# CMU-SAFARI/Genome-on-Diet

Measured on AMD Instinct MI355X. Metric: mapped bases/sec (whole node), HiFi map-hifi k19w19, higher is better.
Workload: dtype int16

## Files before the change

### genome-on-diet_amd/build.py

```python
import os
import re
import subprocess

HERE = os.path.dirname(os.path.abspath(__file__))
LIB = os.path.join(HERE, "libgdiet_hip.so")
SRC = os.path.join(HERE, "csrc", "gdiet_hip.hip")
RES = os.path.join(HERE, "build_resources.txt")

BUDGET = {"_Z21ksw_extd2_wave_kernelILi64ELi0ELb1E": dict(vgprs=96, scratch=0),
          "_Z21ksw_extd2_pipe_kernelILb1E": dict(vgprs=128, scratch=320),
          "_Z20map_post_wave_kernel": dict(vgprs=32, scratch=0),
          "_Z21map_pack_cigar_kernel": dict(vgprs=32, scratch=0),
          "_Z25ksw_backtrack_wave_kernel": dict(vgprs=32, scratch=0),
          "_Z22ksw_exact_match_kernel": dict(vgprs=32, scratch=0),
          "_Z18map_diffstr_kernel": dict(vgprs=32, scratch=0),
          "_Z18fastx_count_kernel": dict(vgprs=32, scratch=0),
          "_Z18fastx_write_kernel": dict(vgprs=32, scratch=0),
          "_Z19fastx_record_kernel": dict(vgprs=32, scratch=0),
          "_Z19fastx_encode_kernel": dict(vgprs=32, scratch=0),
          "_Z19bgzf_inflate_kernel": dict(vgprs=64, scratch=0),
          "_Z19bgzf_deflate_kernel": dict(vgprs=128, scratch=0),
          "_Z17bam_encode_kernel": dict(vgprs=32, scratch=0),
          "_Z17sam_encode_kernel": dict(vgprs=32, scratch=0),
          "_Z17bam_unpack_kernel": dict(vgprs=32, scratch=0),
          "_Z14bam_key_kernel": dict(vgprs=32, scratch=0),
          "_Z17bam_gather_kernel": dict(vgprs=32, scratch=0),
          "_Z14dup_key_kernel": dict(vgprs=32, scratch=0),
          "_Z17dup_decide_kernel": dict(vgprs=32, scratch=0),
          "_Z16dup_apply_kernel": dict(vgprs=32, scratch=0),
          "_Z18cov_scatter_kernel": dict(vgprs=32, scratch=0),
          "_Z17cov_window_kernel": dict(vgprs=32, scratch=0),
          "_Z19pile_scatter_kernel": dict(vgprs=32, scratch=0),
          "_Z16pile_call_kernel": dict(vgprs=32, scratch=0),
          "_Z16pile_site_kernel": dict(vgprs=32, scratch=0)}


def _newest_source():
    m = 0.0
    for root in (os.path.join(HERE, "csrc"), os.path.join(os.path.dirname(HERE), "include")):
        for f in os.listdir(root):
            m = max(m, os.path.getmtime(os.path.join(root, f)))
    return m


def check_resources(text):
    found = {}
    blocks = re.split(r"remark: Function Name: ", text)
    for b in blocks[1:]:
        name = b.split()[0]
        for prefix, lim in BUDGET.items():
            if name.startswith(prefix):
                v = re.search(r"remark:\s+VGPRs: (\d+)", b)
                sc = re.search(r"ScratchSize \[bytes/lane\]: (\d+)", b)
                if v and sc:
                    found[prefix] = (int(v.group(1)), int(sc.group(1)))
                    if int(v.group(1)) > lim["vgprs"] or int(sc.group(1)) > lim["scratch"]:
                        raise RuntimeError("%s: %d VGPRs / %d B scratch per lane, budget %d / %d (genome-on-diet_amd/build.py)"
                                           % (name, int(v.group(1)), int(sc.group(1)), lim["vgprs"], lim["scratch"]))
    missing = [p for p in BUDGET if p not in found]
    if missing:
        raise RuntimeError("no resource report for %s" % missing)
    return found


def build_hip(force=False, verbose=False):
    if not force and os.path.exists(LIB) and os.path.getmtime(LIB) >= _newest_source():
        return LIB
    hipcc = os.environ.get("HIPCC", "/opt/rocm/bin/hipcc")
    cmd = [hipcc, "--offload-arch=gfx950", "-O3", "-std=c++17", "-fPIC", "-shared", "-pthread", "-mllvm", "-amdgpu-sched-strategy=max-ilp",
           "-Rpass-analysis=kernel-resource-usage", "-o", LIB, SRC, "-lz"]
    if verbose:
        print(" ".join(cmd))
    r = subprocess.run(cmd, stderr=subprocess.PIPE, text=True)
    remarks = "\n".join(l for l in r.stderr.split("\n") if "-Rpass-analysis=kernel-resource-usage" in l)
    other = "\n".join(l for l in r.stderr.split("\n") if "-Rpass-analysis=kernel-resource-usage" not in l)
    if r.returncode:
        raise RuntimeError("hipcc failed:\n" + other[-4000:])
    open(RES, "w").write(remarks)
    found = check_resources(remarks)
    if verbose:
        print("register budgets:", found)
    return LIB


if __name__ == "__main__":
    print(build_hip(force=True, verbose=True))
```

### genome-on-diet_amd/csrc/map_kernels.hip.h

```cpp
#pragma once
#include <hip/hip_runtime.h>
#include "map_stages.h"
#include "map_post.h"

struct MapDevOpt {
	int32_t k, w;
	float max_seeds, q_occ_frac;
	int32_t mid_occ, max_max_occ, occ_dist;
	uint32_t max_nb_seeds;
	int64_t flag;
	GdLrVoteOpt vote;
	GdSrVoteOpt sr;
	int32_t is_sr;
	int32_t sort_cap;
	uint32_t seed_lds;
	int32_t prio;
	GdPattern pat;
};
__device__ __forceinline__ void map_set_prio(int p)
{
	if (p == 1) __builtin_amdgcn_s_setprio(1);
	else if (p == 2) __builtin_amdgcn_s_setprio(2);
	else if (p >= 3) __builtin_amdgcn_s_setprio(3);
}


struct MapSeedOut {
	int32_t n_seeds;
	int32_t shift;
	uint32_t tel;
	uint32_t n_mv;
	int64_t n_a;
};

__device__ __forceinline__ unsigned map_sketch2_lds(const uint8_t *str, int len, int w, int k, const GdPattern &P, float max_seeds, GdMini *out, unsigned max_out,
                                                    uint32_t *shift_n, GdMini *win)
{
	unsigned len_crop, total = 0;
	uint32_t cap;
	if (max_seeds < 1) len_crop = (unsigned)((float)max_seeds * len), cap = UINT32_MAX;
	else len_crop = len, cap = (uint32_t)max_seeds;
	for (int shift = 0; shift < P.W; ++shift) {
		const unsigned dl = gd_diet_len(P, len_crop, shift);
		GdEmitCount e = {out + total, 0, cap, max_out - total, false};
		gd_sketch_range<GdEmitCount, true>(str, 0, 0, dl, 0, true, w, k, 0, (unsigned)shift, P, true, e, win, 64);
		if (e.overflow) return ~0u;
		shift_n[shift] = e.n;
		total += e.n;
		if (cap == UINT32_MAX) len_crop = len, cap = e.n;
	}
	return total;
}
__device__ __forceinline__ unsigned map_sketch3_lds(const uint8_t *str, unsigned len, int w, int k, const GdPattern &P, int shift, uint32_t max_nb_seeds, GdMini *out,
                                                    unsigned max_out, unsigned *n_out, GdMini *win)
{
	if (shift < 0) shift = 0;
	const unsigned dl = gd_diet_len(P, len, (unsigned)shift);
	GdEmitCap e = {out, 0, max_nb_seeds, max_out, len, false};
	gd_sketch_range<GdEmitCap, true>(str, 0, 0, dl, 0, true, w, k, 0, (unsigned)shift, P, true, e, win, 64);
	*n_out = e.overflow ? ~0u : e.n;
	return e.ret;
}

__global__ __launch_bounds__(64) void map_seed_kernel(int n_reads, const uint8_t *__restrict__ reads, const int64_t *__restrict__ roff,
                                                      GdIdxView I, MapDevOpt O, const MapReadScratch *__restrict__ sc, GdMini *__restrict__ mv_arena,
                                                      uint64_t *__restrict__ u64_arena, GdSeed *__restrict__ seed_arena, MapSeedOut *__restrict__ out)
{
	extern __shared__ __attribute__((aligned(16))) uint8_t seed_thread_lds[];
	GdMini *win = reinterpret_cast<GdMini *>(seed_thread_lds) + threadIdx.x;
	const int rid = blockIdx.x * blockDim.x + threadIdx.x;
	if (rid >= n_reads) return;
	const uint8_t *str = reads + roff[rid];
	const int len = (int)(roff[rid + 1] - roff[rid]);
	MapSeedOut o;
	o.n_seeds = 0, o.shift = 0, o.tel = (uint32_t)len, o.n_mv = 0, o.n_a = 0;
	if (len <= 0) { out[rid] = o; return; }
	const MapReadScratch S = sc[rid];
	GdMini *mv = mv_arena + S.mv_off;
	uint32_t shift_n[64];
	const unsigned tot = map_sketch2_lds(str, len, O.w, O.k, O.pat, O.max_seeds, mv, S.mv_cap, shift_n, win);
	if (tot == ~0u) { o.n_seeds = -1; out[rid] = o; return; }
	o.shift = (int32_t)gd_get_shift(I, mv, shift_n, O.pat.W);
	unsigned n_mv = 0;
	o.tel = map_sketch3_lds(str, (unsigned)len, O.w, O.k, O.pat, o.shift, O.max_nb_seeds, mv, S.mv_cap, &n_mv, win);
	if (n_mv == ~0u) { o.n_seeds = -1; out[rid] = o; return; }
// ... 313 lines not shown
	GdPostOut P;
	P.qshift = P.tshift = P.mlen = P.blen = P.dp_max = 0, P.n_ambi = 0;
	const int32_t n0 = __builtin_amdgcn_readfirstlane(n_cigar[b]);
	const int32_t sc_b = __builtin_amdgcn_readfirstlane(score[b]);
	const int64_t c0 = coff[b], c1 = coff[b + 1];
	const bool live = sc_b != GD_NEG_INF_SCORE_DEV && n0 > 0 && (int64_t)n0 <= c1 - c0;
	int32_t n_out = n0;
	if (live) {
		uint32_t *cg = (uint32_t *)gdw_uniform_ptr((const uint8_t *)(cig + c0), 0);
		const uint8_t *qseq = gdw_uniform_ptr(qbuf + boxes[b].q_dst, 0), *tseq = gdw_uniform_ptr(tbuf + boxes[b].t_dst, 0);
		uint32_t n_fix = (uint32_t)n0;
		int32_t qshift = 0, tshift = 0;
		if (lane == 0) {
			gdp_fix_cigar(cg, &n_fix, qseq, tseq, &qshift, &tshift);
			n_cigar[b] = (int32_t)n_fix;
		}
		__builtin_amdgcn_fence(__ATOMIC_SEQ_CST, "workgroup");
		const uint32_t n = (uint32_t)__builtin_amdgcn_readfirstlane((int)n_fix);
		n_out = (int32_t)n;
		P.qshift = __builtin_amdgcn_readfirstlane(qshift), P.tshift = __builtin_amdgcn_readfirstlane(tshift);
		__syncthreads();
		qseq += P.qshift, tseq += P.tshift;
		int32_t Si = 0, Sf = 0, MXi = 0, MXf = 0;
		int32_t qoff = 0, toff = 0, blen = 0, mlen = 0;
		uint32_t n_ambi_tot = 0;
		for (uint32_t k = 0; k < n; ++k) {
			const uint32_t c = (uint32_t)__builtin_amdgcn_readfirstlane((int)cg[k]), op = c & 0xf, len = c >> 4;
			if (op == 0) {
				for (uint32_t base = 0; base < len; base += 64) {
					GdpSeg g = {0, GDP_NONE, GDP_NONE, GDP_NONE};
					int cnt2 = 0;
					const uint32_t l = base + lane;
					if (l < len) {
						const int cq = qseq[qoff + l], ct = tseq[toff + l];
						if (ct > 3 || cq > 3) cnt2 = 1;
						else if (ct != cq) cnt2 = 1 << 16;
						const int idx = ct * 5 + cq;
						const int32_t a = idx < 25 ? (int32_t)s_mat[idx] : 0;
						g = gdp_seg_base(a);
					}
#pragma unroll 1
					for (int d = 1; d < 64; d <<= 1) {
						GdpSeg o;
						o.A = __shfl_down(g.A, d), o.B = __shfl_down(g.B, d), o.P = __shfl_down(g.P, d), o.Q = __shfl_down(g.Q, d);
						const int oc = __shfl_down(cnt2, d);
						if (lane + d < 64) g = gdp_seg_join(g, o), cnt2 += oc;
					}
					const int32_t A = __builtin_amdgcn_readfirstlane(g.A), Bc = __builtin_amdgcn_readfirstlane(g.B), Pm = __builtin_amdgcn_readfirstlane(g.P),
					              Qm = __builtin_amdgcn_readfirstlane(g.Q);
					const int c2 = __builtin_amdgcn_readfirstlane(cnt2), na = c2 & 0xffff, nd = c2 >> 16;
					gdp_run_fold(A, Bc, Pm, Qm, Si, Sf, MXi, MXf);
					const uint32_t cnt = len - base < 64 ? len - base : 64;
					blen += (int32_t)cnt - na, mlen += (int32_t)cnt - (na + nd), n_ambi_tot += (uint32_t)na;
				}
				toff += len, qoff += len;
			} else if (op == 1 || op == 2) {
				int na = 0;
				const uint8_t *src = op == 1 ? qseq + qoff : tseq + toff;
				for (uint32_t l0 = 0; l0 < len; l0 += 64) na += __popcll(__ballot(l0 + lane < len && src[l0 + lane] > 3));
				blen += (int32_t)len - na, n_ambi_tot += (uint32_t)na;
				const double tot = gdp_gap_cost(O.q, O.e, O.log_gap, len);
				const int32_t Ti = __builtin_amdgcn_readfirstlane(gdp_gap_int(tot));
				const int32_t Tf = __builtin_amdgcn_readfirstlane(gdp_gap_frac(tot, Ti));
				gdp_run_gap(Ti, Tf, Si, Sf);
				if (op == 1) qoff += len; else toff += len;
			} else if (op == 3) toff += len;
		}
		P.mlen = mlen, P.blen = blen, P.n_ambi = n_ambi_tot;
		P.dp_max = gdp_run_round(MXi, MXf);
	}
	if (lane == 0) {
		post[b] = P;
		if (x_score) x_score[b] = sc_b, x_ncig[b] = n_out;
	}
}


#ifdef GD_SEED_PROF
__device__ unsigned long long gd_seed_prof[8];
#define GD_PROF_T(i) do { const unsigned long long t_ = wall_clock64(); if (lane == 0) atomicAdd(&gd_seed_prof[i], t_ - prof_t); prof_t = t_; } while (0)
#else
#define GD_PROF_T(i) do { } while (0)
#endif
struct GdEmitLane {
	GdMini *out;
	unsigned n, cap;
	__device__ bool operator()(const GdMini &m)
	{
		if (n < cap) out[n] = m;
		++n;
		return false;
	}
};

__device__ __forceinline__ unsigned map_par_sketch_range(const uint8_t *str, unsigned dl, unsigned a, unsigned b, int w, int k, unsigned shift, const GdPattern &P,
                                                         GdMini *tmp, unsigned R, GdMini *dst, unsigned dst_cap, uint32_t cap, unsigned have, GdMini *win)
{
	const unsigned lane = threadIdx.x & 63;
	const unsigned chunk = (b - a + 63) / 64;
	const unsigned i0 = a + lane * chunk, i1 = i0 + chunk < b ? i0 + chunk : b;
	GdEmitLane e = {tmp + (size_t)lane * R, 0, R};
#ifdef GD_SEED_PROF
	unsigned long long prof_t = wall_clock64();
#endif
	if (chunk && i0 < b) gd_sketch_slice<GdEmitLane, true>(str, dl, i0, i1, w, k, 0, shift, P, true, e, win + lane, 64);
	GD_PROF_T(6);
	unsigned incl = e.n;
	for (int d = 1; d < 64; d <<= 1) {
		const unsigned v = __shfl_up(incl, d);
		if ((int)lane >= d) incl += v;
	}
	const unsigned total = have + __shfl(incl, 63), off = have + incl - e.n;
	const unsigned eff = (cap > 0 && total >= cap) ? cap : total;
	bool bad = e.n > R;
	for (unsigned j = 0; j < e.n && !bad; ++j) {
		const unsigned p = off + j;
		if (p >= eff) break;
		if (p < dst_cap) dst[p] = e.out[j];
		else bad = true;
	}
	GD_PROF_T(7);
	return __any(bad) ? ~0u : eff;
}

__device__ __forceinline__ unsigned map_par_sketch(const uint8_t *str, unsigned dl, int w, int k, unsigned shift, const GdPattern &P, GdMini *tmp,
                                                   unsigned R, GdMini *dst, unsigned dst_cap, uint32_t cap, GdMini *win )
{
	if (cap == 0) return map_par_sketch_range(str, dl, 0, dl, w, k, shift, P, tmp, R, dst, dst_cap, 0, 0, win);
	uint64_t l1 = (uint64_t)cap * (uint64_t)(w + 1) / 2;
	l1 += l1 / 4 + (unsigned)(w + k);
	if (l1 >= dl) return map_par_sketch_range(str, dl, 0, dl, w, k, shift, P, tmp, R, dst, dst_cap, cap, 0, win);
	const unsigned n1 = map_par_sketch_range(str, dl, 0, (unsigned)l1, w, k, shift, P, tmp, R, dst, dst_cap, cap, 0, win);
	if (n1 == ~0u || n1 >= cap) return n1;
	__syncthreads();
	return map_par_sketch_range(str, dl, (unsigned)l1, dl, w, k, shift, P, tmp, R, dst, dst_cap, cap, n1, win);
}

__global__ __launch_bounds__(64) void map_seed_wave_kernel(int n_reads, const uint8_t *__restrict__ reads, const int64_t *__restrict__ roff,
                                                           GdIdxView I, MapDevOpt O, const MapReadScratch *__restrict__ sc, GdMini *__restrict__ mv_arena,
                                                           uint64_t *__restrict__ u64_arena, GdSeed *__restrict__ seed_arena, MapSeedOut *__restrict__ out,
                                                           const int32_t *__restrict__ ids )
{
	map_set_prio(O.prio);
	if ((int)blockIdx.x >= n_reads) return;
	const int rid = ids ? ids[blockIdx.x] : (int)blockIdx.x;
	const unsigned lane = threadIdx.x;
	const uint8_t *str = reads + roff[rid];
	const int len = (int)(roff[rid + 1] - roff[rid]);
	MapSeedOut o;
	o.n_seeds = 0, o.shift = 0, o.tel = (uint32_t)len, o.n_mv = 0, o.n_a = 0;
	if (len <= 0) { if (lane == 0) out[rid] = o; return; }
	const MapReadScratch S = sc[rid];
	GdMini *mv = mv_arena + S.mv_off;
	GdMini *tmp = (GdMini *)(u64_arena + S.u64_off);
	GdSeed *seeds = seed_arena + S.seed_off;
	const unsigned R = S.mv_cap / 64;
	extern __shared__ __attribute__((aligned(16))) uint8_t seed_lds[];
	GdMini *win = reinterpret_cast<GdMini *>(seed_lds);
#ifdef GD_SEED_PROF
	unsigned long long prof_t = wall_clock64();
#endif
	unsigned len_crop, total = 0;
	uint32_t cap;
	if (O.max_seeds < 1) len_crop = (unsigned)((float)O.max_seeds * len), cap = UINT32_MAX;
	else len_crop = (unsigned)len, cap = (uint32_t)O.max_seeds;
	uint32_t shift_n[64];
	bool bad = false;
	for (int shift = 0; shift < O.pat.W; ++shift) {
		const unsigned dl = gd_diet_len(O.pat, len_crop, (unsigned)shift);
		const unsigned n = map_par_sketch(str, dl, O.w, O.k, (unsigned)shift, O.pat, tmp, R, mv + total, S.mv_cap - total, cap == UINT32_MAX ? 0u : cap, win);
		__syncthreads();
		if (n == ~0u) { bad = true; break; }
		shift_n[shift] = n, total += n;
		if (cap == UINT32_MAX) len_crop = (unsigned)len, cap = n;
	}
	if (bad) { o.n_seeds = -1; if (lane == 0) out[rid] = o; return; }
	GD_PROF_T(0);
	{
		unsigned best = 0, base = 0;
		for (int i = 0; i < O.pat.W; ++i) {
			unsigned cur = 0;
			for (unsigned j = lane; j < shift_n[i]; j += 64) {
				uint64_t st;
				cur += gd_idx_get(I, mv[base + j].x >> 8, &st);
			}
			for (int d = 32; d > 0; d >>= 1) cur += __shfl_xor(cur, d);
			if (cur > best) o.shift = i, best = cur;
			base += shift_n[i];
		}
	}
	__syncthreads();
	GD_PROF_T(1);
	unsigned n_mv;
	{
		const unsigned dl = gd_diet_len(O.pat, (unsigned)len, (unsigned)o.shift);
		n_mv = map_par_sketch(str, dl, O.w, O.k, (unsigned)o.shift, O.pat, tmp, R, mv, S.mv_cap, O.max_nb_seeds == UINT32_MAX ? 0u : O.max_nb_seeds, win);
		__syncthreads();
		if (n_mv == ~0u) { o.n_seeds = -1; if (lane == 0) out[rid] = o; return; }
		if (O.max_nb_seeds != UINT32_MAX && O.max_nb_seeds > 0 && n_mv == O.max_nb_seeds) o.tel = (uint32_t)(mv[n_mv - 1].y >> 1);
	}
	GD_PROF_T(2);
	if (O.q_occ_frac > 0.0f && (int64_t)n_mv > (int64_t)O.mid_occ && O.mid_occ > 0) {
		uint64_t *srt = reinterpret_cast<uint64_t *>(seed_lds);
		bool need = true;
		{
			const unsigned nb = (unsigned)(O.seed_lds / sizeof(uint32_t)) >= 8192u ? 8192u : 4096u;
			uint32_t *cnt = reinterpret_cast<uint32_t *>(seed_lds);
			for (unsigned i = lane; i < nb; i += 64) cnt[i] = 0;
			__syncthreads();
			for (unsigned i = lane; i < n_mv; i += 64) atomicAdd(&cnt[(unsigned)((mv[i].x >> 8) * 0x9E3779B97F4A7C15ull >> 40) & (nb - 1)], 1u);
			__syncthreads();
			bool over = false;
			for (unsigned i = lane; i < nb; i += 64) over |= cnt[i] > (uint32_t)O.mid_occ;
			need = __any(over);
			__syncthreads();
		}
		if (need && n_mv <= (unsigned)O.sort_cap) {
			unsigned P2 = 64;
			while (P2 < n_mv) P2 <<= 1;
			for (unsigned i = lane; i < P2; i += 64) srt[i] = i < n_mv ? mv[i].x : UINT64_MAX;
			__syncthreads();
			for (unsigned kk = 2; kk <= P2; kk <<= 1)
				for (unsigned jj = kk >> 1; jj > 0; jj >>= 1) {
					for (unsigned i = lane; i < P2; i += 64) {
						const unsigned ixj = i ^ jj;
						if (ixj > i) {
							const uint64_t a = srt[i], b = srt[ixj];
							const bool up = (i & kk) == 0;
							if ((a > b) == up) srt[i] = b, srt[ixj] = a;
						}
					}
					__syncthreads();
				}
			bool hit = false;
			for (unsigned i = lane; i + (unsigned)O.mid_occ < n_mv; i += 64) hit |= srt[i] == srt[i + (unsigned)O.mid_occ];
			need = __any(hit);
		}
		if (need) {
			unsigned nn = 0;
			if (lane == 0) nn = gd_mz_flt(mv, n_mv, O.mid_occ, O.q_occ_frac, u64_arena + S.u64_off);
			__syncthreads();
			n_mv = __shfl(nn, 0);
		}
	}
	GD_PROF_T(3);
	const bool in_lds = (size_t)n_mv * sizeof(GdSeed) <= (size_t)O.seed_lds;
	GdSeed *work = in_lds ? reinterpret_cast<GdSeed *>(seed_lds) : seeds;
	for (unsigned j = lane; j < n_mv; j += 64) gd_collect_probe(I, mv[j], work[j]);
	__syncthreads();
	GD_PROF_T(4);
	int n_m0 = 0;
	bool any_high = false;
	for (unsigned b0 = 0; b0 < n_mv; b0 += 64) {
		const unsigned j = b0 + lane;
		GdSeed sd;
		sd.n = 0;
		if (j < n_mv) sd = work[j];
		const bool keep = j < n_mv && sd.n != 0;
		const uint64_t m = __ballot(keep);
		any_high |= keep && (int32_t)sd.n > O.mid_occ;
		__syncthreads();
		if (keep) work[n_m0 + __popcll(m & ((1ull << lane) - 1))] = sd;
		n_m0 += __popcll(m);
		__syncthreads();
	}
	if (__any(any_high)) {
		if (O.occ_dist > 0 && O.max_max_occ > O.mid_occ) {
			if (lane == 0) gd_seed_select(n_m0, work, len, O.mid_occ, O.max_max_occ, O.occ_dist);
		} else
			for (int j = (int)lane; j < n_m0; j += 64)
				if ((int32_t)work[j].n > O.mid_occ) work[j].flt = 1;
		__syncthreads();
	}
	int n_kept = 0;
	int64_t n_a = 0;
	for (int b0 = 0; b0 < n_m0; b0 += 64) {
		const int j = b0 + (int)lane;
		GdSeed sd;
		sd.n = 0, sd.flt = 1;
		if (j < n_m0) sd = work[j];
		const bool keep = j < n_m0 && !sd.flt;
		const uint64_t m = __ballot(keep);
		if (keep) n_a += sd.n;
// ... 15 lines not shown
```

### genome-on-diet_amd/csrc/map_pipeline.hip.h

```cpp
#pragma once
#include <atomic>
#include <memory>
#include <cstddef>
#include <chrono>
#include <thread>
#include <mutex>
#include "map_host.h"
#include "map_plan.h"
#include "map_index.h"
#include "map_kernels.hip.h"

struct gdiet_index {
	GdIndex h;
	void *d_tkey = nullptr, *d_tval = nullptr, *d_pos = nullptr, *d_S = nullptr;
	GdIdxView dview;
	bool host_tables = true;
	uint32_t *d_cnt_sorted = nullptr;
	uint64_t n_pos = 0;
	uint32_t *d_seq_len = nullptr;
	uint64_t *d_seq_off = nullptr;
	std::mutex seq_mu;
	std::vector<const char *> info_names;
	std::vector<uint32_t> info_lens;
	int64_t open_counts[6] = {0, 0, 0, 0, 0, 0};
// ... 373 lines not shown
}

struct GdMapCall {
	gdiet_ctx *ctx;
	const gdiet_index *ix;
	const GdMapOpt &O;
	const GdBatchView &B;
	int32_t *n_regs;
	gdiet_reg_t **regs;
	GdStageTrace mark;
	double t0 = 0;
	MapDevOpt D;
	bool is_sr = false, sr_dev = false;
	std::vector<MapReadScratch> sc;
	GdSeedClasses cls;
	MapSeedOut *so = nullptr;
	std::vector<int64_t> hoff;
	GdBoxTables T;
	size_t nbp = 64;
	int64_t *d_coff = nullptr;
	int32_t *d_ex = nullptr, *d_score = nullptr, *d_ncig = nullptr;
	int32_t *h_score = nullptr, *h_ncig = nullptr;
	const GdPostOut *h_post = nullptr;
	uint32_t *h_cig = nullptr;
	std::vector<int64_t> poff{0};
};

static void gd_lap(GdMapCall &c, int stage) { c.ctx->stage_s[stage] += gd_now() - c.t0, c.t0 = gd_now(); }

static int gd_scratch_grow(GdMapCall &c, bool full)
{
	gdiet_ctx *ctx = c.ctx;
	const int n = c.B.n;
	const uint64_t tot = gd_scratch_layout(n, c.B.roff, c.O.w, c.O.pat, c.O.max_seeds, full, c.sc.data());
	int rc;
	if ((rc = gd_grow(ctx, ctx->m_sc, sizeof(MapReadScratch) * n))) return rc;
	if ((rc = gd_grow(ctx, ctx->m_mv, sizeof(GdMini) * tot))) return rc;
	if ((rc = gd_grow(ctx, ctx->m_u64, sizeof(uint64_t) * 2 * tot))) return rc;
	if ((rc = gd_grow(ctx, ctx->m_seed, sizeof(GdSeed) * tot))) return rc;
	GD_HIP(hipMemcpyAsync(ctx->m_sc.p, c.sc.data(), sizeof(MapReadScratch) * n, hipMemcpyHostToDevice, ctx->stream));
	return GDIET_OK;
}

static int gd_stage_setup(GdMapCall &c)
{
	gdiet_ctx *ctx = c.ctx;
	const GdMapOpt &O = c.O;
	const int n = c.B.n;
	int rc;
	c.sc.resize(n);
	if ((rc = gd_scratch_grow(c, false))) return rc;
	if ((rc = gd_grow(ctx, ctx->m_seedout, sizeof(MapSeedOut) * n))) return rc;
	if ((rc = gd_grow(ctx, ctx->m_voteout, sizeof(MapVoteOut) * n))) return rc;
	if ((rc = gd_grow(ctx, ctx->m_hitoff, sizeof(int64_t) * (n + 1)))) return rc;
	MapDevOpt &D = c.D;
	D.k = O.k, D.w = O.w, D.max_seeds = O.max_seeds, D.q_occ_frac = O.q_occ_frac, D.mid_occ = O.mid_occ, D.max_max_occ = O.max_max_occ, D.occ_dist = O.occ_dist;
	D.max_nb_seeds = (O.flag & GD_F_FRAG_MODE) ? (O.max_frag_len == 0 ? 800u : (uint32_t)O.max_frag_len) : UINT32_MAX;
	D.flag = O.flag, D.pat = O.pat;
	D.vote.vt_dis = O.vt_dis, D.vote.vt_nb_loc = O.vt_nb_loc, D.vote.bw = O.bw, D.vote.vt_cov = O.vt_cov, D.vote.vt_f = O.vt_f;
	D.vote.vt_df1 = O.vt_df1, D.vote.vt_df2 = O.vt_df2, D.vote.k = O.k;
	c.is_sr = (O.flag & GD_F_SR) != 0;
	D.is_sr = c.is_sr;
	D.prio = 2;
	gd_seed_classes(O.pat, O.w, n, c.B.roff, c.cls);
	D.sort_cap = c.cls.sort_cap;
	D.sr.min_cnt = O.min_cnt, D.sr.rec_threshold_frac = O.rec_threshold_frac, D.sr.bw_frac = O.bw_frac, D.sr.bw_min = O.bw_min, D.sr.bw_max = O.bw_max;
	D.sr.af_max_loc = O.af_max_loc, D.sr.max_nb_seeds = D.max_nb_seeds, D.sr.frag_mode = (O.flag & GD_F_FRAG_MODE) != 0;
	c.sr_dev = c.is_sr && ctx->sr_boxes_on_device && (int64_t)n * std::min<int64_t>(O.af_max_loc, GDM_MAX_VT) < ((int64_t)1 << 28);
	return GDIET_OK;
}

static int gd_stage_seed(GdMapCall &c)
{
	gdiet_ctx *ctx = c.ctx;
	const gdiet_index *ix = c.ix;
	const GdMapOpt &O = c.O;
	const GdBatchView &B = c.B;
	MapDevOpt &D = c.D;
	const int n = B.n;
	hipStream_t s = ctx->stream;
	int rc;
	if ((rc = gd_host_grow(ctx, ctx->h_seedout, sizeof(MapSeedOut) * (size_t)n))) return rc;
	MapSeedOut *so = c.so = (MapSeedOut *)ctx->h_seedout.p;
	const size_t seed_lds = gd_seed_lds_bytes(O.w, D.sort_cap);
	D.seed_lds = (uint32_t)seed_lds;
	if (seed_lds > 64 * 1024) GD_HIP(hipFuncSetAttribute((const void *)map_seed_wave_kernel, hipFuncAttributeMaxDynamicSharedMemorySize, (int)seed_lds));
	for (int attempt = 0; attempt < 2; ++attempt) {
		if (ctx->seed_thread_kernel == 1 || (ctx->seed_thread_kernel == 0 && (B.roff[n] - B.roff[0]) / n < 1024))
			hipLaunchKernelGGL(map_seed_kernel, dim3((n + 63) / 64), dim3(64), (size_t)O.w * 64 * sizeof(GdMini), s, n, B.d_reads, B.d_roff, ix->dview, D, (const MapReadScratch *)ctx->m_sc.p,
			                   (GdMini *)ctx->m_mv.p, (uint64_t *)ctx->m_u64.p, (GdSeed *)ctx->m_seed.p, (MapSeedOut *)ctx->m_seedout.p);
		else if (!c.cls.classes.empty()) {
			if ((rc = gd_grow(ctx, ctx->m_seedids, sizeof(int32_t) * (size_t)n))) return rc;
			GD_HIP(hipMemcpyAsync(ctx->m_seedids.p, c.cls.ids.data(), sizeof(int32_t) * (size_t)n, hipMemcpyHostToDevice, s));
			int at = 0;
			for (const auto &cls : c.cls.classes) {
				MapDevOpt Dc = D;
				Dc.sort_cap = cls.first;
				const size_t lds_c = gd_seed_lds_bytes(O.w, cls.first);
				Dc.seed_lds = (uint32_t)lds_c;
				hipLaunchKernelGGL(map_seed_wave_kernel, dim3(cls.second), dim3(64), lds_c, s, cls.second, B.d_reads, B.d_roff, ix->dview, Dc, (const MapReadScratch *)ctx->m_sc.p,
				                   (GdMini *)ctx->m_mv.p, (uint64_t *)ctx->m_u64.p, (GdSeed *)ctx->m_seed.p, (MapSeedOut *)ctx->m_seedout.p, (const int32_t *)ctx->m_seedids.p + at);
				at += cls.second;
			}
		} else
			hipLaunchKernelGGL(map_seed_wave_kernel, dim3(n), dim3(64), seed_lds, s, n, B.d_reads, B.d_roff, ix->dview, D, (const MapReadScratch *)ctx->m_sc.p,
			                   (GdMini *)ctx->m_mv.p, (uint64_t *)ctx->m_u64.p, (GdSeed *)ctx->m_seed.p, (MapSeedOut *)ctx->m_seedout.p, (const int32_t *)nullptr);
		GD_HIP(hipGetLastError());
		GD_HIP(hipMemcpyAsync(so, ctx->m_seedout.p, sizeof(MapSeedOut) * n, hipMemcpyDeviceToHost, s));
		GD_HIP(gd_stream_wait(ctx, s));
		bool overflow = false;
		for (int i = 0; i < n; ++i) overflow |= so[i].n_seeds < 0;
		if (!overflow) break;
		if (attempt == 1) { ctx->err = "minimizer scratch overflow even with the hard bound"; return GDIET_E_NOMEM; }
		++gd_scratch_retries;
		if ((rc = gd_scratch_grow(c, true))) return rc;
	}
	return GDIET_OK;
}

static int gd_seed_export(GdMapCall &c, GdSeedExport &sx)
{
	gdiet_ctx *ctx = c.ctx;
	const int n = c.B.n;
	const MapSeedOut *so = c.so;
	hipStream_t s = ctx->stream;
	sx.out.assign(so, so + n);
	int64_t tot_seeds = 0;
	for (int i = 0; i < n; ++i) tot_seeds += so[i].n_seeds > 0 ? so[i].n_seeds : 0;
	sx.seeds.resize((size_t)tot_seeds);
	int64_t at = 0;
	for (int i = 0; i < n; ++i)
		if (so[i].n_seeds > 0) {
			GD_HIP(hipMemcpyAsync(sx.seeds.data() + at, (const GdSeed *)ctx->m_seed.p + c.sc[i].seed_off, sizeof(GdSeed) * (size_t)so[i].n_seeds, hipMemcpyDeviceToHost, s));
			at += so[i].n_seeds;
		}
	GD_HIP(gd_stream_wait(ctx, s));
	return GDIET_OK;
}

static int gd_stage_vote(GdMapCall &c)
{
	gdiet_ctx *ctx = c.ctx;
	const gdiet_index *ix = c.ix;
	const GdBatchView &B = c.B;
	const int n = B.n;
	hipStream_t s = ctx->stream;
	std::vector<int64_t> &hoff = c.hoff;
	int rc;
	hoff.assign(n + 1, 0);
	for (int i = 0; i < n; ++i) {
		hoff[i + 1] = hoff[i] + (c.so[i].n_seeds > 0 ? c.so[i].n_a : 0);
	}
	if ((rc = gd_grow(ctx, ctx->m_hits, sizeof(GdLoc) * 3 * (size_t)(hoff[n] + 1)))) return rc;
	GD_HIP(hipMemcpyAsync(ctx->m_hitoff.p, hoff.data(), sizeof(int64_t) * (n + 1), hipMemcpyHostToDevice, s));
	const int spread = (B.roff[n] - B.roff[0]) / n >= 1024;
	if (spread == 1 && ctx->vote_wave) {
		int64_t max_hits = 0;
		for (int i = 0; i < n; ++i) max_hits = std::max(max_hits, hoff[i + 1] - hoff[i]);
		unsigned vote_cap = 256;
		while (vote_cap < MAP_VOTE_CAP && (int64_t)vote_cap < max_hits) vote_cap <<= 1;
		if (sizeof(GdLoc) * (size_t)vote_cap + sizeof(GdVt) * GDM_MAX_VT + 64 > 64 * 1024)
			GD_HIP(hipFuncSetAttribute((const void *)map_vote_wave_kernel, hipFuncAttributeMaxDynamicSharedMemorySize, (int)(sizeof(GdLoc) * (size_t)vote_cap)));
		hipLaunchKernelGGL(map_vote_wave_kernel, dim3(n), dim3(64), sizeof(GdLoc) * (size_t)vote_cap, s, n, B.d_roff, ix->dview, c.D, (const MapReadScratch *)ctx->m_sc.p,
		                   (const GdSeed *)ctx->m_seed.p, (const MapSeedOut *)ctx->m_seedout.p, (const int64_t *)ctx->m_hitoff.p, (GdLoc *)ctx->m_hits.p,
		                   (MapVoteOut *)ctx->m_voteout.p, vote_cap);
	} else
		hipLaunchKernelGGL(map_vote_kernel, dim3(spread ? n : (n + 63) / 64), dim3(64), 0, s, n, B.d_roff, ix->dview, c.D, (const MapReadScratch *)ctx->m_sc.p,
		                   (const GdSeed *)ctx->m_seed.p, (const MapSeedOut *)ctx->m_seedout.p, (const int64_t *)ctx->m_hitoff.p, (GdLoc *)ctx->m_hits.p,
		                   (MapVoteOut *)ctx->m_voteout.p, spread);
	GD_HIP(hipGetLastError());
	return GDIET_OK;
}

static int gd_aux_layout(GdMapCall &c)
{
	gdiet_ctx *ctx = c.ctx;
	const int nb = c.T.nb;
	c.nbp = ((size_t)std::max(nb, 1) + 63) & ~(size_t)63;
	int rc;
	if ((rc = gd_grow(ctx, ctx->m_aux, sizeof(int64_t) * (nb + 1) + sizeof(int32_t) * 3 * c.nbp + 1024))) return rc;
	c.d_coff = (int64_t *)ctx->m_aux.p;
// ... 908 lines not shown
```

Measured before the change: 2.499 billion.

## Replace per-lane chunked minimizer sketch with wave-cooperative tiled sketch

The seed wave kernel now computes minimizers cooperatively across the wave: 64 consecutive positions per step, with k-mers built from ballots and bit reversal and a log-depth sliding-window minimum held in LDS ring buffers. This replaces the old scheme where each lane sketched its own chunk into a global scratch buffer and the results were compacted with a prefix scan. The goal is to remove per-lane serial window work, scratch traffic and the extra copy. The shift-selection and final sketch passes are merged into one loop, shift counts move to LDS, and occupancy is hinted at 8 waves per EU. Tie handling inside windows now needs extra serial rescans, and the scratch budget allowed for this kernel is raised.

Result: faster. 2.626 billion, median of 6 (+5.1%).

```diff
diff --git a/genome-on-diet_amd/build.py b/genome-on-diet_amd/build.py
--- a/genome-on-diet_amd/build.py
+++ b/genome-on-diet_amd/build.py
@@ -11,6 +11,7 @@
           "_Z21ksw_extd2_pipe_kernelILb1E": dict(vgprs=128, scratch=320),
           "_Z20map_post_wave_kernel": dict(vgprs=32, scratch=0),
           "_Z21map_pack_cigar_kernel": dict(vgprs=32, scratch=0),
+          "_Z20map_seed_wave_kernel": dict(vgprs=64, scratch=1152),
           "_Z25ksw_backtrack_wave_kernel": dict(vgprs=32, scratch=0),
           "_Z22ksw_exact_match_kernel": dict(vgprs=32, scratch=0),
           "_Z18map_diffstr_kernel": dict(vgprs=32, scratch=0),
diff --git a/genome-on-diet_amd/csrc/map_kernels.hip.h b/genome-on-diet_amd/csrc/map_kernels.hip.h
--- a/genome-on-diet_amd/csrc/map_kernels.hip.h
+++ b/genome-on-diet_amd/csrc/map_kernels.hip.h
@@ -1,6 +1,7 @@
 #pragma once
 #include <hip/hip_runtime.h>
 #include "map_stages.h"
+#include "map_tile_sketch.h"
 #include "map_post.h"
 
 struct MapDevOpt {
@@ -480,61 +481,14 @@
 #else
 #define GD_PROF_T(i) do { } while (0)
 #endif
-struct GdEmitLane {
-	GdMini *out;
-	unsigned n, cap;
-	__device__ bool operator()(const GdMini &m)
-	{
-		if (n < cap) out[n] = m;
-		++n;
-		return false;
-	}
+
+struct MapSeedLds {
+	GdTileLds tile;
+	uint32_t shift_n[64];
 };
-
-__device__ __forceinline__ unsigned map_par_sketch_range(const uint8_t *str, unsigned dl, unsigned a, unsigned b, int w, int k, unsigned shift, const GdPattern &P,
-                                                         GdMini *tmp, unsigned R, GdMini *dst, unsigned dst_cap, uint32_t cap, unsigned have, GdMini *win)
-{
-	const unsigned lane = threadIdx.x & 63;
-	const unsigned chunk = (b - a + 63) / 64;
-	const unsigned i0 = a + lane * chunk, i1 = i0 + chunk < b ? i0 + chunk : b;
-	GdEmitLane e = {tmp + (size_t)lane * R, 0, R};
-#ifdef GD_SEED_PROF
-	unsigned long long prof_t = wall_clock64();
-#endif
-	if (chunk && i0 < b) gd_sketch_slice<GdEmitLane, true>(str, dl, i0, i1, w, k, 0, shift, P, true, e, win + lane, 64);
-	GD_PROF_T(6);
-	unsigned incl = e.n;
-	for (int d = 1; d < 64; d <<= 1) {
-		const unsigned v = __shfl_up(incl, d);
-		if ((int)lane >= d) incl += v;
-	}
-	const unsigned total = have + __shfl(incl, 63), off = have + incl - e.n;
-	const unsigned eff = (cap > 0 && total >= cap) ? cap : total;
-	bool bad = e.n > R;
-	for (unsigned j = 0; j < e.n && !bad; ++j) {
-		const unsigned p = off + j;
-		if (p >= eff) break;
-		if (p < dst_cap) dst[p] = e.out[j];
-		else bad = true;
-	}
-	GD_PROF_T(7);
-	return __any(bad) ? ~0u : eff;
-}
-
-__device__ __forceinline__ unsigned map_par_sketch(const uint8_t *str, unsigned dl, int w, int k, unsigned shift, const GdPattern &P, GdMini *tmp,
-                                                   unsigned R, GdMini *dst, unsigned dst_cap, uint32_t cap, GdMini *win )
-{
-	if (cap == 0) return map_par_sketch_range(str, dl, 0, dl, w, k, shift, P, tmp, R, dst, dst_cap, 0, 0, win);
-	uint64_t l1 = (uint64_t)cap * (uint64_t)(w + 1) / 2;
-	l1 += l1 / 4 + (unsigned)(w + k);
-	if (l1 >= dl) return map_par_sketch_range(str, dl, 0, dl, w, k, shift, P, tmp, R, dst, dst_cap, cap, 0, win);
-	const unsigned n1 = map_par_sketch_range(str, dl, 0, (unsigned)l1, w, k, shift, P, tmp, R, dst, dst_cap, cap, 0, win);
-	if (n1 == ~0u || n1 >= cap) return n1;
-	__syncthreads();
-	return map_par_sketch_range(str, dl, (unsigned)l1, dl, w, k, shift, P, tmp, R, dst, dst_cap, cap, n1, win);
-}
-
-__global__ __launch_bounds__(64) void map_seed_wave_kernel(int n_reads, const uint8_t *__restrict__ reads, const int64_t *__restrict__ roff,
+static inline size_t gd_seed_wave_lds_bytes(int cap) { return sizeof(MapSeedLds) > (size_t)cap * sizeof(uint64_t) ? sizeof(MapSeedLds) : (size_t)cap * sizeof(uint64_t); }
+
+__global__ __launch_bounds__(64) __attribute__((amdgpu_waves_per_eu(8))) void map_seed_wave_kernel(int n_reads, const uint8_t *__restrict__ reads, const int64_t *__restrict__ roff,
                                                            GdIdxView I, MapDevOpt O, const MapReadScratch *__restrict__ sc, GdMini *__restrict__ mv_arena,
                                                            uint64_t *__restrict__ u64_arena, GdSeed *__restrict__ seed_arena, MapSeedOut *__restrict__ out,
                                                            const int32_t *__restrict__ ids )
@@ -550,53 +504,52 @@
 	if (len <= 0) { if (lane == 0) out[rid] = o; return; }
 	const MapReadScratch S = sc[rid];
 	GdMini *mv = mv_arena + S.mv_off;
-	GdMini *tmp = (GdMini *)(u64_arena + S.u64_off);
 	GdSeed *seeds = seed_arena + S.seed_off;
-	const unsigned R = S.mv_cap / 64;
 	extern __shared__ __attribute__((aligned(16))) uint8_t seed_lds[];
-	GdMini *win = reinterpret_cast<GdMini *>(seed_lds);
+	MapSeedLds *SL = reinterpret_cast<MapSeedLds *>(seed_lds);
 #ifdef GD_SEED_PROF
 	unsigned long long prof_t = wall_clock64();
 #endif
-	unsigned len_crop, total = 0;
+	unsigned len_crop, total = 0, n_mv = 0;
 	uint32_t cap;
 	if (O.max_seeds < 1) len_crop = (unsigned)((float)O.max_seeds * len), cap = UINT32_MAX;
 	else len_crop = (unsigned)len, cap = (uint32_t)O.max_seeds;
-	uint32_t shift_n[64];
-	bool bad = false;
-	for (int shift = 0; shift < O.pat.W; ++shift) {
+	const int W = O.pat.W;
+#pragma unroll 1
+	for (int pass = 0; pass <= W; ++pass) {
+		int shift = pass;
+		if (pass == W) {
+			GD_PROF_T(0);
+			unsigned best = 0, base = 0;
+#pragma unroll 1
+			for (int i = 0; i < W; ++i) {
+				unsigned cur = 0;
+				const unsigned n_i = SL->shift_n[i];
+#pragma unroll 1
+				for (unsigned j = lane; j < n_i; j += 64) {
+					uint64_t st;
+					cur += gd_idx_get(I, mv[base + j].x >> 8, &st);
+				}
+				for (int d = 32; d > 0; d >>= 1) cur += __shfl_xor(cur, d);
+				if (cur > best) o.shift = i, best = cur;
+				base += n_i;
+			}
+			__syncthreads();
+			GD_PROF_T(1);
+			shift = o.shift, len_crop = (unsigned)len, total = 0, cap = O.max_nb_seeds;
+		}
 		const unsigned dl = gd_diet_len(O.pat, len_crop, (unsigned)shift);
-		const unsigned n = map_par_sketch(str, dl, O.w, O.k, (unsigned)shift, O.pat, tmp, R, mv + total, S.mv_cap - total, cap == UINT32_MAX ? 0u : cap, win);
+		const unsigned n = gd_tile_sketch(str, dl, O.w, O.k, 0, (unsigned)shift, O.pat, true, mv + total, S.mv_cap - total, cap == UINT32_MAX ? 0u : cap, &SL->tile);
 		__syncthreads();
-		if (n == ~0u) { bad = true; break; }
-		shift_n[shift] = n, total += n;
-		if (cap == UINT32_MAX) len_crop = (unsigned)len, cap = n;
-	}
-	if (bad) { o.n_seeds = -1; if (lane == 0) out[rid] = o; return; }
-	GD_PROF_T(0);
-	{
-		unsigned best = 0, base = 0;
-		for (int i = 0; i < O.pat.W; ++i) {
-			unsigned cur = 0;
-			for (unsigned j = lane; j < shift_n[i]; j += 64) {
-				uint64_t st;
-				cur += gd_idx_get(I, mv[base + j].x >> 8, &st);
-			}
-			for (int d = 32; d > 0; d >>= 1) cur += __shfl_xor(cur, d);
-			if (cur > best) o.shift = i, best = cur;
-			base += shift_n[i];
+		if (n == ~0u) { o.n_seeds = -1; if (lane == 0) out[rid] = o; return; }
+		if (pass == W) n_mv = n;
+		else {
+			SL->shift_n[pass] = n, total += n;
+			if (cap == UINT32_MAX) len_crop = (unsigned)len, cap = n;
 		}
 	}
 	__syncthreads();
-	GD_PROF_T(1);
-	unsigned n_mv;
-	{
-		const unsigned dl = gd_diet_len(O.pat, (unsigned)len, (unsigned)o.shift);
-		n_mv = map_par_sketch(str, dl, O.w, O.k, (unsigned)o.shift, O.pat, tmp, R, mv, S.mv_cap, O.max_nb_seeds == UINT32_MAX ? 0u : O.max_nb_seeds, win);
-		__syncthreads();
-		if (n_mv == ~0u) { o.n_seeds = -1; if (lane == 0) out[rid] = o; return; }
-		if (O.max_nb_seeds != UINT32_MAX && O.max_nb_seeds > 0 && n_mv == O.max_nb_seeds) o.tel = (uint32_t)(mv[n_mv - 1].y >> 1);
-	}
+	if (O.max_nb_seeds != UINT32_MAX && O.max_nb_seeds > 0 && n_mv == O.max_nb_seeds) o.tel = (uint32_t)(mv[n_mv - 1].y >> 1);
 	GD_PROF_T(2);
 	if (O.q_occ_frac > 0.0f && (int64_t)n_mv > (int64_t)O.mid_occ && O.mid_occ > 0) {
 		uint64_t *srt = reinterpret_cast<uint64_t *>(seed_lds);
diff --git a/genome-on-diet_amd/csrc/map_pipeline.hip.h b/genome-on-diet_amd/csrc/map_pipeline.hip.h
--- a/genome-on-diet_amd/csrc/map_pipeline.hip.h
+++ b/genome-on-diet_amd/csrc/map_pipeline.hip.h
@@ -479,7 +479,7 @@
 	int rc;
 	if ((rc = gd_host_grow(ctx, ctx->h_seedout, sizeof(MapSeedOut) * (size_t)n))) return rc;
 	MapSeedOut *so = c.so = (MapSeedOut *)ctx->h_seedout.p;
-	const size_t seed_lds = gd_seed_lds_bytes(O.w, D.sort_cap);
+	const size_t seed_lds = gd_seed_wave_lds_bytes(D.sort_cap);
 	D.seed_lds = (uint32_t)seed_lds;
 	if (seed_lds > 64 * 1024) GD_HIP(hipFuncSetAttribute((const void *)map_seed_wave_kernel, hipFuncAttributeMaxDynamicSharedMemorySize, (int)seed_lds));
 	for (int attempt = 0; attempt < 2; ++attempt) {
@@ -493,7 +493,7 @@
 			for (const auto &cls : c.cls.classes) {
 				MapDevOpt Dc = D;
 				Dc.sort_cap = cls.first;
-				const size_t lds_c = gd_seed_lds_bytes(O.w, cls.first);
+				const size_t lds_c = gd_seed_wave_lds_bytes(cls.first);
 				Dc.seed_lds = (uint32_t)lds_c;
 				hipLaunchKernelGGL(map_seed_wave_kernel, dim3(cls.second), dim3(64), lds_c, s, cls.second, B.d_reads, B.d_roff, ix->dview, Dc, (const MapReadScratch *)ctx->m_sc.p,
 				                   (GdMini *)ctx->m_mv.p, (uint64_t *)ctx->m_u64.p, (GdSeed *)ctx->m_seed.p, (MapSeedOut *)ctx->m_seedout.p, (const int32_t *)ctx->m_seedids.p + at);
diff --git a/genome-on-diet_amd/csrc/map_tile_sketch.h b/genome-on-diet_amd/csrc/map_tile_sketch.h
--- /dev/null
+++ b/genome-on-diet_amd/csrc/map_tile_sketch.h
@@ -0,0 +1,268 @@
+#pragma once
+#include "map_stages.h"
+
+#define GDT_LEVELS 7
+#define GDT_RING 128
+
+struct GdTileLds {
+	uint64_t lx[GDT_LEVELS][GDT_RING];
+	uint32_t lo[GDT_LEVELS][GDT_RING];
+	uint64_t mx[GDT_RING];
+	uint32_t mo[GDT_RING];
+	uint32_t cnt[64];
+	int32_t ones_loc[GDM_MAX_ONES];
+};
+
+#if defined(__HIP_DEVICE_COMPILE__)
+#define GDT_NL 1
+#define GDT_EACH_LANE for (unsigned lane = threadIdx.x & 63, gdt_once_ = 1; gdt_once_; gdt_once_ = 0)
+#define GDT_LI 0
+#define GDT_SYNC() __syncthreads()
+#define GDT_BALLOT(dst_, arr_) dst_ = __ballot(arr_[0])
+#define GDT_NOUNROLL _Pragma("unroll 1")
+#else
+#define GDT_NL 64
+#define GDT_EACH_LANE for (unsigned lane = 0; lane < 64; ++lane)
+#define GDT_LI lane
+#define GDT_SYNC() ((void)0)
+#define GDT_NOUNROLL
+#define GDT_BALLOT(dst_, arr_) do { dst_ = 0; for (unsigned q_ = 0; q_ < 64; ++q_) dst_ |= (uint64_t)(arr_[q_] != 0) << q_; } while (0)
+#endif
+#define GDT_V(a_) a_[GDT_LI]
+
+GDM_HD uint64_t gdt_brev64(uint64_t v)
+{
+#if defined(__HIP_DEVICE_COMPILE__)
+	return __brevll(v);
+#else
+	v = (v >> 1 & 0x5555555555555555ull) | (v & 0x5555555555555555ull) << 1;
+	v = (v >> 2 & 0x3333333333333333ull) | (v & 0x3333333333333333ull) << 2;
+	v = (v >> 4 & 0x0f0f0f0f0f0f0f0full) | (v & 0x0f0f0f0f0f0f0f0full) << 4;
+	return __builtin_bswap64(v);
+#endif
+}
+
+GDM_HD uint32_t gdt_spread16(uint32_t a)
+{
+	a = (a | a << 8) & 0x00ff00ffu;
+	a = (a | a << 4) & 0x0f0f0f0fu;
+	a = (a | a << 2) & 0x33333333u;
+	return (a | a << 1) & 0x55555555u;
+}
+
+GDM_HD int gdt_popc64(uint64_t v)
+{
+#if defined(__HIP_DEVICE_COMPILE__)
+	return __popcll(v);
+#else
+	return __builtin_popcountll(v);
+#endif
+}
+
+GDM_HDI unsigned gd_tile_sketch(const uint8_t *str, unsigned dl, int w, int k, uint32_t rid, unsigned shift, const GdPattern &P, bool final_ge,
+                                GdMini *dst, unsigned dst_cap, uint32_t cap, GdTileLds *L)
+{
+	const uint64_t mask = (1ULL << 2 * k) - 1, yhi = (uint64_t)rid << 32;
+	const uint32_t kmask = (1u << k) - 1;
+	const unsigned ones = (unsigned)P.ones, W = (unsigned)P.W, loc0 = (unsigned)P.ones_loc[0];
+	const bool one_1 = ones == 1;
+	const int full = w + k - 1;
+	int ptop = 0;
+	while ((2 << ptop) <= w) ++ptop;
+	const unsigned rest = (unsigned)w - (1u << ptop);
+	const uint32_t lim = cap ? cap : UINT32_MAX;
+	GDT_EACH_LANE {
+		GDT_NOUNROLL
+		for (int p = 0; p <= ptop; ++p) {
+			L->lx[p][lane] = L->lx[p][lane + 64] = UINT64_MAX;
+			L->lo[p][lane] = L->lo[p][lane + 64] = 0;
+		}
+		L->mx[lane] = L->mx[lane + 64] = UINT64_MAX;
+		L->mo[lane] = L->mo[lane + 64] = 0;
+		if (!one_1)
+			GDT_NOUNROLL
+			for (unsigned j = 0; j < ones; ++j) L->ones_loc[j] = P.ones_loc[j];
+	}
+	GDT_SYNC();
+	uint64_t pb0 = 0, pb1 = 0;
+	unsigned lc = 0, have = 0;
+	uint8_t fbad[GDT_NL];
+	GDT_EACH_LANE GDT_V(fbad) = 0;
+	GDT_NOUNROLL
+	for (unsigned t0 = 0; t0 < dl; t0 += 64) {
+		uint8_t c[GDT_NL], f0[GDT_NL], f1[GDT_NL], fn[GDT_NL];
+		uint32_t ylo[GDT_NL];
+		GDT_EACH_LANE {
+			const unsigned i = t0 + lane;
+			unsigned real;
+			if (one_1) real = i * W + loc0 + shift;
+			else {
+				const unsigned iq = i / ones;
+				real = iq * W + (unsigned)L->ones_loc[i - iq * ones] + shift;
+			}
+			uint8_t b = 4;
+			if (i < dl) { b = str[real]; if (b > 4) b = 4; }
+			GDT_V(c) = b, GDT_V(ylo) = real << 1;
+			GDT_V(f0) = b & 1, GDT_V(f1) = (b >> 1) & 1, GDT_V(fn) = b >> 2;
+		}
+		uint64_t b0, b1, bN;
+		GDT_BALLOT(b0, f0);
+		GDT_BALLOT(b1, f1);
+		GDT_BALLOT(bN, fn);
+		int l[GDT_NL], lp[GDT_NL];
+		uint64_t x[GDT_NL], cx[GDT_NL];
+		uint32_t co[GDT_NL];
+		GDT_EACH_LANE {
+			const uint64_t le = lane == 63 ? ~0ull : (2ull << lane) - 1;
+			const uint64_t m = bN & le, mp = bN & (le >> 1);
+			GDT_V(l) = m ? (int)lane - (63 - __builtin_clzll(m)) : (int)(lc + lane + 1);
+			GDT_V(lp) = mp ? (int)lane - 1 - (63 - __builtin_clzll(mp)) : (int)(lc + lane);
+			const uint64_t v0 = b0 << (63 - lane) | (pb0 >> lane) >> 1, v1 = b1 << (63 - lane) | (pb1 >> lane) >> 1;
+			const uint32_t r0 = (uint32_t)gdt_brev64(v0) & kmask, r1 = (uint32_t)gdt_brev64(v1) & kmask;
+			const uint64_t fw = (uint64_t)(gdt_spread16(r0 >> 16) | gdt_spread16(r1 >> 16) << 1) << 32 | (gdt_spread16(r0 & 0xffff) | gdt_spread16(r1 & 0xffff) << 1);
+			uint64_t rv = gdt_brev64(fw);
+			rv = (rv >> 1 & 0x5555555555555555ull) | (rv & 0x5555555555555555ull) << 1;
+			rv = ~(rv >> (64 - 2 * k)) & mask;
+			uint64_t xi = UINT64_MAX;
+			uint32_t z = 0;
+			if (GDT_V(c) < 4 && GDT_V(l) >= k && fw != rv) {
+				z = fw < rv ? 0 : 1;
+				xi = gd_hash64(z ? rv : fw, mask) << 8 | (uint64_t)k;
+			}
+			GDT_V(ylo) |= z;
+			GDT_V(x) = GDT_V(cx) = xi, GDT_V(co) = 0;
+			const unsigned slot = (t0 + lane) & (GDT_RING - 1);
+			L->lx[0][slot] = xi, L->lo[0][slot] = GDT_V(ylo);
+		}
+		GDT_SYNC();
+		GDT_NOUNROLL
+		for (int p = 1; p <= ptop; ++p) {
+			const unsigned d = 1u << (p - 1);
+			GDT_EACH_LANE {
+				const unsigned j = (t0 + lane - d) & (GDT_RING - 1), slot = (t0 + lane) & (GDT_RING - 1);
+				const uint64_t xb = L->lx[p - 1][j];
+				const uint32_t ob = (p == 1 ? 0u : L->lo[p - 1][j]) + d * 0x101u;
+				const uint32_t oa = GDT_V(co);
+				GDT_V(co) = ((xb < GDT_V(cx) ? ob : oa) & 0xffu) | ((xb <= GDT_V(cx) ? ob : oa) & 0xff00u);
+				if (xb < GDT_V(cx)) GDT_V(cx) = xb;
+				if (p < ptop || rest) L->lx[p][slot] = GDT_V(cx), L->lo[p][slot] = GDT_V(co);
+			}
+			GDT_SYNC();
+		}
+		uint64_t px[GDT_NL];
+		uint32_t po[GDT_NL];
+		GDT_EACH_LANE {
+			const unsigned slot = (t0 + lane) & (GDT_RING - 1);
+			if (rest) {
+				const unsigned j = (t0 + lane - rest) & (GDT_RING - 1);
+				const uint64_t xb = L->lx[ptop][j];
+				const uint32_t ob = L->lo[ptop][j] + rest * 0x101u, oa = GDT_V(co);
+				GDT_V(co) = ((xb < GDT_V(cx) ? ob : oa) & 0xffu) | ((xb <= GDT_V(cx) ? ob : oa) & 0xff00u);
+				if (xb < GDT_V(cx)) GDT_V(cx) = xb;
+			}
+			L->mx[slot] = GDT_V(cx), L->mo[slot] = GDT_V(co);
+		}
+		GDT_SYNC();
+		uint8_t ep[GDT_NL], et[GDT_NL];
+		GDT_EACH_LANE {
+			const unsigned j = (t0 + lane - 1) & (GDT_RING - 1);
+			GDT_V(px) = L->mx[j], GDT_V(po) = L->mo[j];
+			const bool vp = GDT_V(px) != UINT64_MAX, vc = GDT_V(cx) != UINT64_MAX;
+			const bool left = vp && !(GDT_V(x) <= GDT_V(px)) && (GDT_V(po) & 0xffu) == (unsigned)(w - 1);
+			bool e;
+			if (GDT_V(c) >= 4) e = GDT_V(lp) >= full;
+			else if (GDT_V(x) <= GDT_V(px)) e = GDT_V(l) >= full + 1;
+			else e = left && GDT_V(l) >= full;
+			GDT_V(ep) = vp && e && t0 + lane < dl;
+			const bool t3 = left && GDT_V(l) >= full && vc, t4 = GDT_V(l) == full && vc;
+			GDT_V(et) = (t3 || t4) && (GDT_V(co) & 0xffu) != (GDT_V(co) >> 8) && t0 + lane < dl;
+		}
+		uint64_t be, bt;
+		GDT_BALLOT(be, ep);
+		GDT_BALLOT(bt, et);
+		unsigned total;
+		if (bt == 0) {
+			GDT_EACH_LANE {
+				if (GDT_V(ep)) {
+					const unsigned p = have + (unsigned)gdt_popc64(be & ((1ull << lane) - 1));
+					if (p < lim) {
+						if (p < dst_cap) {
+							const unsigned a = (t0 + lane - 1 - (GDT_V(po) & 0xffu)) & (GDT_RING - 1);
+							dst[p].x = GDT_V(px), dst[p].y = yhi | L->lo[0][a];
+						} else GDT_V(fbad) = 1;
+					}
+				}
+			}
+			total = (unsigned)gdt_popc64(be);
+		} else {
+			GDT_EACH_LANE {
+				unsigned n = GDT_V(ep);
+				if (GDT_V(et)) {
+					const int i = (int)(t0 + lane), ac = i - (int)(GDT_V(co) & 0xffu);
+					const int j1 = GDT_V(l) == full ? i - 1 : i;
+					GDT_NOUNROLL
+					for (int j = i - w + 1; j <= j1; ++j)
+						if (j >= 0 && j != ac && L->lx[0][j & (GDT_RING - 1)] == GDT_V(cx)) ++n;
+				}
+				L->cnt[lane] = n;
+			}
+			GDT_SYNC();
+			total = 0;
+			GDT_NOUNROLL
+			for (unsigned q = 0; q < 64; ++q) total += L->cnt[q];
+			GDT_EACH_LANE {
+				unsigned p = have;
+				GDT_NOUNROLL
+				for (unsigned q = 0; q < lane; ++q) p += L->cnt[q];
+				if (GDT_V(ep)) {
+					if (p < lim) {
+						if (p < dst_cap) {
+							const unsigned a = (t0 + lane - 1 - (GDT_V(po) & 0xffu)) & (GDT_RING - 1);
+							dst[p].x = GDT_V(px), dst[p].y = yhi | L->lo[0][a];
+						} else GDT_V(fbad) = 1;
+					}
+					++p;
+				}
+				if (GDT_V(et)) {
+					const int i = (int)(t0 + lane), ac = i - (int)(GDT_V(co) & 0xffu);
+					const int j1 = GDT_V(l) == full ? i - 1 : i;
+					GDT_NOUNROLL
+					for (int j = i - w + 1; j <= j1; ++j)
+						if (j >= 0 && j != ac && L->lx[0][j & (GDT_RING - 1)] == GDT_V(cx)) {
+							if (p < lim) {
+								if (p < dst_cap) dst[p].x = GDT_V(cx), dst[p].y = yhi | L->lo[0][j & (GDT_RING - 1)];
+								else GDT_V(fbad) = 1;
+							}
+							++p;
+						}
+				}
+			}
+			GDT_SYNC();
+		}
+		have += total;
+		if (have >= lim) {
+			have = lim;
+			break;
+		}
+		if (t0 + 64 >= dl) {
+			uint8_t ff[GDT_NL];
+			GDT_EACH_LANE GDT_V(ff) = t0 + lane == dl - 1 && (final_ge ? GDT_V(l) >= full : GDT_V(l) > full) && GDT_V(cx) != UINT64_MAX;
+			uint64_t bf;
+			GDT_BALLOT(bf, ff);
+			GDT_EACH_LANE {
+				if (GDT_V(ff)) {
+					if (have < dst_cap) {
+						const unsigned a = (t0 + lane - (GDT_V(co) & 0xffu)) & (GDT_RING - 1);
+						dst[have].x = GDT_V(cx), dst[have].y = yhi | L->lo[0][a];
+					} else GDT_V(fbad) = 1;
+				}
+			}
+			if (bf) ++have;
+		}
+		pb0 = b0, pb1 = b1;
+		lc = bN ? (unsigned)__builtin_clzll(bN) : lc + 64;
+	}
+	uint64_t bb;
+	GDT_BALLOT(bb, fbad);
+	return bb ? ~0u : have;
+}
```
